# unilight/jatts

Hardware: AMD Instinct MI355X
Metric: audio samples/sec (22.05 kHz) + RTF, FastSpeech2+HiFi-GAN (higher is better)
Workload: dtype f32 (emulated: 3 exact bf16 terms per operand, 7 MFMA products, f32 accumulate; attention / norms / duration predictor exact f32); 1 GPU; FastSpeech2(JSUT conformer 4+4, adim 384)+HiFi-GAN v1 22k, 64 utts x 128 phonemes x 6 frames per GPU; hop=256, parallelism=dp1 (utterance sharding, int16 PCM all-gather)

## Files before the change

### jatts_amd/csrc/resunit_emul16_impl.h

```cpp
#pragma once
#include <type_traits>

#include "resunit_emul_impl.h"

#ifndef JATTS_U16_ROWS
#define JATTS_U16_ROWS 1
#endif
#ifndef JATTS_U16_DIAG
#define JATTS_U16_DIAG 0
#endif

namespace {

struct acc2x4 { f32x4 big, small; };
template <typename T> struct Acc16 { typedef f32x4 type; };
template <> struct Acc16<bf3p<7>> { typedef acc2x4 type; };
__device__ __forceinline__ void acc16_set(f32x4& a, int i, float v) { a[i] = v; }
__device__ __forceinline__ void acc16_set(acc2x4& a, int i, float v) { a.small[i] = v; a.big[i] = 0.f; }
__device__ __forceinline__ void acc16_finish(f32x4&) {}
__device__ __forceinline__ void acc16_finish(acc2x4& a) { a.small = a.big + a.small; }
__device__ __forceinline__ f32x4& acc16_val(f32x4& a) { return a; }
__device__ __forceinline__ f32x4& acc16_val(acc2x4& a) { return a.small; }

template <int P> __device__ __forceinline__ void mma16p(const bf3px8<7>& a, const bf3px8<7>& b, acc2x4& c) {
  if constexpr (P == 0) c.small = __builtin_amdgcn_mfma_f32_16x16x32_bf16(a.b1, b.b2, c.small, 0, 0, 0);
  if constexpr (P == 1) c.small = __builtin_amdgcn_mfma_f32_16x16x32_bf16(a.b2, b.b0, c.small, 0, 0, 0);
  if constexpr (P == 2) c.small = __builtin_amdgcn_mfma_f32_16x16x32_bf16(a.b0, b.b2, c.small, 0, 0, 0);
  if constexpr (P == 3) c.small = __builtin_amdgcn_mfma_f32_16x16x32_bf16(a.b1, b.b1, c.small, 0, 0, 0);
  if constexpr (P == 4) c.small = __builtin_amdgcn_mfma_f32_16x16x32_bf16(a.b1, b.b0, c.small, 0, 0, 0);
  if constexpr (P == 5) c.small = __builtin_amdgcn_mfma_f32_16x16x32_bf16(a.b0, b.b1, c.small, 0, 0, 0);
  if constexpr (P == 6) c.big = __builtin_amdgcn_mfma_f32_16x16x32_bf16(a.b0, b.b0, c.big, 0, 0, 0);
}
template <int P> __device__ __forceinline__ void mma16p(const bf3px8<6>& a, const bf3px8<6>& b, f32x4& c) {
  if constexpr (P == 0) c = __builtin_amdgcn_mfma_f32_16x16x32_bf16(a.b2, b.b0, c, 0, 0, 0);
  if constexpr (P == 1) c = __builtin_amdgcn_mfma_f32_16x16x32_bf16(a.b0, b.b2, c, 0, 0, 0);
  if constexpr (P == 2) c = __builtin_amdgcn_mfma_f32_16x16x32_bf16(a.b1, b.b1, c, 0, 0, 0);
  if constexpr (P == 3) c = __builtin_amdgcn_mfma_f32_16x16x32_bf16(a.b1, b.b0, c, 0, 0, 0);
  if constexpr (P == 4) c = __builtin_amdgcn_mfma_f32_16x16x32_bf16(a.b0, b.b1, c, 0, 0, 0);
  if constexpr (P == 5) c = __builtin_amdgcn_mfma_f32_16x16x32_bf16(a.b0, b.b0, c, 0, 0, 0);
}
template <typename T> struct NProd;
template <int NP> struct NProd<bf3p<NP>> { static constexpr int value = NP; };

template <typename T, int NF>
struct WStream16 {
  typedef typename Elem<T>::vec8 V8;
  V8 ra[NF];
  const T* wl;
  int kc_stride;
  int tap_stride;
  __device__ __forceinline__ void bind(const T* w, int KC32, int NFR16, int nf0, int lane) {
    wl = w + (size_t)nf0 * 512 + (size_t)lane * 8;
    kc_stride = NFR16 * 512;
    tap_stride = KC32 * kc_stride;
  }
  __device__ __forceinline__ void fetch(int tap, int kc) {
    const T* p = wl + (size_t)tap * tap_stride + (size_t)kc * kc_stride;
#pragma unroll
    for (int f = 0; f < NF; ++f) ra[f] = Vec8IO<T>::ldg(p + f * 512);
  }
};

template <typename T, int NF, int NT>
__device__ __forceinline__ void pair16(typename Acc16<T>::type (&acc)[NF][NT], const typename Elem<T>::vec8& a, typename Elem<T>::vec8 (&rb)[NT], int f_, int t0_) {
  constexpr int NP = NProd<T>::value;
  auto& c0 = acc[f_][t0_];
  auto& c1 = acc[f_][t0_ + 1];
  mma16p<0>(a, rb[t0_], c0); mma16p<0>(a, rb[t0_ + 1], c1);
  mma16p<1>(a, rb[t0_], c0); mma16p<1>(a, rb[t0_ + 1], c1);
  mma16p<2>(a, rb[t0_], c0); mma16p<2>(a, rb[t0_ + 1], c1);
  mma16p<3>(a, rb[t0_], c0); mma16p<3>(a, rb[t0_ + 1], c1);
  mma16p<4>(a, rb[t0_], c0); mma16p<4>(a, rb[t0_ + 1], c1);
  mma16p<5>(a, rb[t0_], c0); mma16p<5>(a, rb[t0_ + 1], c1);
  if constexpr (NP == 7) { mma16p<6>(a, rb[t0_], c0); mma16p<6>(a, rb[t0_ + 1], c1); }
}

template <typename T, int NF, int NT>
__device__ __forceinline__ void row16(typename Acc16<T>::type (&acc)[NF][NT], const typename Elem<T>::vec8& a, typename Elem<T>::vec8 (&rb)[NT], int f_) {
  constexpr int NP = NProd<T>::value;
#pragma unroll
  for (int t = 0; t < NT; ++t) mma16p<0>(a, rb[t], acc[f_][t]);
#pragma unroll
  for (int t = 0; t < NT; ++t) mma16p<1>(a, rb[t], acc[f_][t]);
#pragma unroll
  for (int t = 0; t < NT; ++t) mma16p<2>(a, rb[t], acc[f_][t]);
#pragma unroll
  for (int t = 0; t < NT; ++t) mma16p<3>(a, rb[t], acc[f_][t]);
#pragma unroll
  for (int t = 0; t < NT; ++t) mma16p<4>(a, rb[t], acc[f_][t]);
#pragma unroll
  for (int t = 0; t < NT; ++t) mma16p<5>(a, rb[t], acc[f_][t]);
  if constexpr (NP == 7) {
#pragma unroll
    for (int t = 0; t < NT; ++t) mma16p<6>(a, rb[t], acc[f_][t]);
  }
}

template <typename T, int NF, int NT>
__device__ __forceinline__ void step16(typename Acc16<T>::type (&acc)[NF][NT], typename Elem<T>::vec8 (&ra)[NF], typename Elem<T>::vec8 (&rb)[NT], const T* pa,
                                       const char* pb, int pitch) {
  static_assert(NT % 2 == 0, "column fragments come in pairs");
  constexpr bool ROWS16 = JATTS_U16_ROWS != 0;
#pragma unroll
  for (int f = 0; f < NF; ++f) {
    if (f < NF - 1 && ROWS16) {
      row16<T, NF, NT>(acc, ra[f], rb, f);
      __builtin_amdgcn_sched_barrier(0);
    } else {
#pragma unroll
      for (int tp = 0; tp < NT; tp += 2) {
        pair16<T, NF, NT>(acc, ra[f], rb, f, tp);
        if (f == NF - 1 && !(JATTS_U16_DIAG & 1)) {
          rb[tp] = Vec8IO<T>::lds(pb + (size_t)(tp * 16) * pitch);
          rb[tp + 1] = Vec8IO<T>::lds(pb + (size_t)((tp + 1) * 16) * pitch);
        }
        __builtin_amdgcn_sched_barrier(0);
      }
    }
    if (!(JATTS_U16_DIAG & 2)) ra[f] = Vec8IO<T>::ldg(pa + f * 512);
    __builtin_amdgcn_sched_barrier(0);
  }
}

template <typename T, int NF, int NT, int KCS>
__device__ __forceinline__ void conv16(typename Acc16<T>::type (&acc)[NF][NT], WStream16<T, NF>& ws, int kc0, int k_w, int dil, const char* act, int pitch,
                                       int col0, int lane, const T* tail) {
  typedef typename Elem<T>::vec8 V8;
  const int steps = k_w * KCS;
  const char* bbase = act + (size_t)(col0 + (lane & 15)) * pitch + (size_t)(lane >> 4) * 48;
  const T* abase = ws.wl + (size_t)kc0 * ws.kc_stride;
  V8 rb[NT];
#pragma unroll
  for (int t = 0; t < NT; ++t) rb[t] = Vec8IO<T>::lds(bbase + (size_t)(t * 16) * pitch);
  __builtin_amdgcn_sched_barrier(0);
  if (!tail) tail = abase + (size_t)(k_w - 1) * ws.tap_stride + (size_t)(KCS - 1) * ws.kc_stride;
  int tap = 0, kk = 0;
  for (int s = 0; s < steps; ++s) {
    int nkk = kk + 1;
    const bool wrap = nkk == KCS;
    nkk = wrap ? 0 : nkk;
    const int ntap = tap + (wrap ? 1 : 0);
    const bool last = s + 1 >= steps;
    const T* pa = last ? tail : abase + (size_t)ntap * ws.tap_stride + (size_t)nkk * ws.kc_stride;
    const char* pb = bbase + (size_t)((last ? tap : ntap) * dil) * pitch + (size_t)((last ? kk : nkk) * 4) * 48;
    step16<T, NF, NT>(acc, ws.ra, rb, pa, pb, pitch);
    tap = ntap;
    kk = nkk;
  }
}

template <typename T, int C, int WGCOLS, int WN, int WT, int OCC, bool KSPLIT = false, bool RREG = false, bool SLIDE = false>
__global__ __launch_bounds__(WN* WT * 64, OCC) void resunit_emul16_kernel(jatts_resunit_desc d, unsigned long long* trace, unsigned trace_cap,
                                                                         unsigned bias_off) {
  typedef typename Elem<T>::vec8 V8;
  extern __shared__ __attribute__((aligned(16))) char smem[];
  constexpr int NF = C / (WN * 16), NT = WGCOLS / (WT * 16);
  constexpr int KC32 = C / 32, NFR16 = C / 16;
  constexpr int pitch = C * 6 + 16;
  constexpr int pitch_x = KSPLIT ? (C / 2) * 6 + 16 : pitch;
  constexpr int pitch_t = C * 6;
  constexpr int NTHR = WN * WT * 64;
  static_assert(NF * WN * 16 == C && NT * WT * 16 == WGCOLS && C % 32 == 0, "tile shape");
  static_assert(sizeof(T) == 6, "bf3 is three packed bf16");
  static_assert(!(KSPLIT && RREG), "the residual registers go with the one-piece x tile");
  static_assert(!KSPLIT || KC32 % 2 == 0, "channel halves are whole K-steps");
  constexpr int MAXI = RREG ? (WGCOLS * (C / 8) + NTHR - 1) / NTHR : 1;
  f32x8 xk[MAXI];
  JATTS_TRACE_BEGIN(trace, trace_cap, blockIdx.x + blockIdx.y * gridDim.x);
  const int K = d.k_w, dil = d.dil;
  const int p2 = (K - 1) / 2, p1 = p2 * dil;
  const int tt_out = WGCOLS - 2 * p2;

  int b, t0;
  int64_t f_seq = 0, f_end = 0;
  if constexpr (!SLIDE) {
    int bx = blockIdx.x;
    b = blockIdx.y;
    if (ragged_is_1d(d.rg) && !ragged_locate(d.rg, tt_out, blockIdx.x, b, bx)) return;
    t0 = bx * tt_out;
  } else {
    const int c0 = d.rg.cu_rows[0];
    const int64_t total = (int64_t)(d.rg.cu_rows[d.rg.n_seq] - c0) * d.rg.len_mul;
    const int64_t per = (total + gridDim.x - 1) / gridDim.x;
    const int64_t f = (int64_t)blockIdx.x * per;
    if (f >= total) return;
    f_end = min(total, f + per);
    b = find_seq(d.rg.cu_rows, d.rg.n_seq, c0 + (int)(f / d.rg.len_mul));
    f_seq = (int64_t)(d.rg.cu_rows[b] - c0) * d.rg.len_mul;
    t0 = (int)(f - f_seq);
  }
  const int lane = threadIdx.x & 63, wave = threadIdx.x >> 6;
  const int wn = wave / WT, wt = wave % WT;
  const int g4 = lane >> 4;
  const int col0 = wt * NT * 16;
  const int nf0 = wn * NF;

  const int rx = WGCOLS + 2 * p1;
  char* xs = smem;
  char* hs = smem;
  float* bs = reinterpret_cast<float*>(smem + bias_off);
  char* tl = smem + bias_off - (SLIDE ? (K - 1) * pitch_t : 0);
  for (int u = threadIdx.x; u < 2 * C; u += NTHR) bs[u] = u < C ? d.b1[u] : d.b2[u - C];

  WStream16<T, NF> ws;
  typename Acc16<T>::type acc[NF][NT];
  auto bias_acc = [&](const float* bv) {
#pragma unroll
    for (int f = 0; f < NF; ++f) {
      const f32x4 bb = *reinterpret_cast<const f32x4*>(bv + (nf0 + f) * 16 + 4 * g4);
#pragma unroll
      for (int t = 0; t < NT; ++t)
#pragma unroll
        for (int e = 0; e < 4; ++e) acc16_set(acc[f][t], e, bb[e]);
    }
  };
  auto finish_acc = [&]() {
#pragma unroll
    for (int f = 0; f < NF; ++f)
#pragma unroll
      for (int t = 0; t < NT; ++t) acc16_finish(acc[f][t]);
  };
  auto to_planes = [&](f32x8 v) {
    lrelu8(v, d.slope);
    V8 o;
    bf3_split8(v, o);
    return o;
  };
  const float* x = (const float*)d.x;
  bool slide = false;
  for (bool first = true;; first = false) {
    unsigned tid = threadIdx.x;
    if constexpr (SLIDE) asm volatile("" : "+v"(tid));
    const int row_b = d.rg.cu_rows[b];
    const int L = (d.rg.cu_rows[b + 1] - row_b) * d.rg.len_mul;
    if constexpr (!SLIDE) {
      if (t0 >= L) return;
    }
    const int64_t seq_row0 = (int64_t)row_b * d.rg.len_mul;
    const int off = slide ? 2 * p2 : 0;
    const int nout = slide ? WGCOLS : tt_out;
    int nvalid = min(nout, L - t0);
    if constexpr (SLIDE) {
      nvalid = (int)min((int64_t)nvalid, f_end - f_seq - t0);
      if (!first) __syncthreads();
    }

    ws.bind((const T*)d.w1, KC32, NFR16, nf0, lane);
    ws.fetch(0, 0);
    const int pos0 = t0 - p2 + off - p1;
    if constexpr (!KSPLIT) {
      constexpr int UPR = C / 8;
      constexpr int UB = 8;
      const int total = rx * UPR;
      if constexpr (RREG) {
        const int r_in = p1 + p2 - off, n_in = nout * UPR;
#pragma unroll
        for (int j = 0; j < MAXI; ++j) {
          const int v = tid + j * NTHR;
          const int ro = v / UPR, cu = v - ro * UPR;
          const int pos = t0 + ro;
          if (v < n_in && pos < L) xk[j] = Vec8IO<float>::ldg(x + (seq_row0 + pos) * (int64_t)C + cu * 8);
          else xk[j] = f32x8{0, 0, 0, 0, 0, 0, 0, 0};
        }
        const int n_halo = (rx - nout) * UPR;
        for (int base = tid; base < n_halo; base += NTHR * UB) {
          f32x8 v[UB];
#pragma unroll
          for (int j = 0; j < UB; ++j) {
            const int u = base + j * NTHR;
            int r = u / UPR;
            const int cu = u - r * UPR;
            if (r >= r_in) r += nout;
            const int pos = pos0 + r;
            if (u < n_halo && pos >= 0 && pos < L) v[j] = Vec8IO<float>::ldg(x + (seq_row0 + pos) * (int64_t)C + cu * 8);
            else v[j] = f32x8{0, 0, 0, 0, 0, 0, 0, 0};
          }
#pragma unroll
          for (int j = 0; j < UB; ++j) {
            const int u = base + j * NTHR;
            if (u >= n_halo) continue;
            int r = u / UPR;
            const int cu = u - r * UPR;
            if (r >= r_in) r += nout;
            Vec8IO<T>::sts(xs + (size_t)r * pitch + (size_t)cu * 48, to_planes(v[j]));
          }
        }
#pragma unroll
        for (int j = 0; j < MAXI; ++j) {
          const int v = tid + j * NTHR;
          if (v >= n_in) continue;
          const int ro = v / UPR, cu = v - ro * UPR;
          Vec8IO<T>::sts(xs + (size_t)(r_in + ro) * pitch + (size_t)cu * 48, to_planes(xk[j]));
        }
      } else {
        constexpr int UBX = ((WGCOLS + 64) * UPR + NTHR - 1) / NTHR;
        for (int base = tid; base < total; base += NTHR * UBX) {
          f32x8 v[UBX];
#pragma unroll
          for (int j = 0; j < UBX; ++j) {
            const int u = base + j * NTHR;
            const int r = u / UPR, cu = u - r * UPR;
            const int pos = pos0 + r;
            if (u < total && pos >= 0 && pos < L) v[j] = Vec8IO<float>::ldg(x + (seq_row0 + pos) * (int64_t)C + cu * 8);
            else v[j] = f32x8{0, 0, 0, 0, 0, 0, 0, 0};
          }
#pragma unroll
          for (int j = 0; j < UBX; ++j) {
            const int u = base + j * NTHR;
            if (u >= total) continue;
            const int r = u / UPR, cu = u - r * UPR;
            Vec8IO<T>::sts(xs + (size_t)r * pitch + (size_t)cu * 48, to_planes(v[j]));
          }
        }
      }
      __syncthreads();
      JATTS_STAMP(2);
      bias_acc(bs);
      conv16<T, NF, NT, KC32>(acc, ws, 0, K, dil, xs, pitch, col0, lane, (const T*)d.w2 + (size_t)nf0 * 512 + (size_t)lane * 8);
    } else {
      constexpr int UPR = C / 16;
      constexpr int MAXU = ((WGCOLS + 64) * UPR + NTHR - 1) / NTHR;
      const int total = rx * UPR;
      f32x8 xv[MAXU];
      auto load_half = [&](int half) {
#pragma unroll
        for (int j = 0; j < MAXU; ++j) {
          const int u = tid + j * NTHR;
          const int r = u / UPR, cu = u - r * UPR;
          const int pos = pos0 + r;
          if (u < total && pos >= 0 && pos < L) xv[j] = Vec8IO<float>::ldg(x + (seq_row0 + pos) * (int64_t)C + half * (C / 2) + cu * 8);
          else xv[j] = f32x8{0, 0, 0, 0, 0, 0, 0, 0};
        }
      };
      auto store_half = [&]() {
#pragma unroll
        for (int j = 0; j < MAXU; ++j) {
          const int u = tid + j * NTHR;
          if (u < total) Vec8IO<T>::sts(xs + (size_t)(u / UPR) * pitch_x + (size_t)(u % UPR) * 48, to_planes(xv[j]));
        }
      };
      load_half(0);
      store_half();
      load_half(1);
      __syncthreads();
      JATTS_STAMP(2);
      bias_acc(bs);
      conv16<T, NF, NT, KC32 / 2>(acc, ws, 0, K, dil, xs, pitch_x, col0, lane, ws.wl + (size_t)(KC32 / 2) * ws.kc_stride);
      lds_barrier();
      store_half();
      lds_barrier();
      conv16<T, NF, NT, KC32 / 2>(acc, ws, KC32 / 2, K, dil, xs, pitch_x, col0, lane, (const T*)d.w2 + (size_t)nf0 * 512 + (size_t)lane * 8);
    }
    finish_acc();
    JATTS_STAMP(3);

    lds_barrier();
    JATTS_STAMP(10);
    if (SLIDE && slide) {
      for (int u = tid; u < (K - 1) * (C / 8); u += NTHR) {
        const int r = u / (C / 8), cu = u % (C / 8);
        Vec8IO<T>::sts(hs + (size_t)r * pitch + (size_t)cu * 48, Vec8IO<T>::lds(tl + (size_t)r * pitch_t + (size_t)cu * 48));
      }
    } else {
      for (int u = tid; u < (K - 1) * (C / 8); u += NTHR) {
        const int r = WGCOLS + u / (C / 8), cu = u % (C / 8);
        V8 z;
#pragma unroll
        for (int e = 0; e < 8; ++e) z.b0[e] = z.b1[e] = z.b2[e] = (bf16)0.f;
        Vec8IO<T>::sts(hs + (size_t)r * pitch + (size_t)cu * 48, z);
      }
    }
#pragma unroll
    for (int t = 0; t < NT; ++t) {
      const int col = col0 + t * 16 + (lane & 15);
      const int pos = t0 - p2 + off + col;
      const float keep = (pos >= 0 && pos < L) ? 1.f : 0.f;
#pragma unroll
      for (int f = 0; f < NF; ++f) {
        const int n0 = (nf0 + f) * 16 + 4 * g4;
        float v[4];
#pragma unroll
        for (int e = 0; e < 4; ++e) {
          const float a = acc16_val(acc[f][t])[e] * keep;
          v[e] = fmaxf(a, a * d.slope);
        }
        bf16x4 q0, q1, q2;
        bf3_split4(v, q0, q1, q2);
        char* p = hs + (size_t)(col + off) * pitch + (size_t)(n0 >> 3) * 48 + (size_t)(n0 & 4) * 2;
        *reinterpret_cast<bf16x4*>(p) = q0;
        *reinterpret_cast<bf16x4*>(p + 16) = q1;
        *reinterpret_cast<bf16x4*>(p + 32) = q2;
      }
    }
    JATTS_STAMP(12);
    lds_barrier();
    JATTS_STAMP(4);

    bias_acc(bs + C);
    ws.bind((const T*)d.w2, KC32, NFR16, nf0, lane);
    conv16<T, NF, NT, KC32>(acc, ws, 0, K, 1, hs, pitch, col0, lane, nullptr);
    finish_acc();
    JATTS_STAMP(5);

    __syncthreads();
    if constexpr (SLIDE) {
      for (int u = tid; u < (K - 1) * (C / 8); u += NTHR) {
        const int r = u / (C / 8), cu = u % (C / 8);
        Vec8IO<T>::sts(tl + (size_t)r * pitch_t + (size_t)cu * 48, Vec8IO<T>::lds(hs + (size_t)(nout + r) * pitch + (size_t)cu * 48));
      }
    }
    char* ys = smem;
#pragma unroll
    for (int t = 0; t < NT; ++t) {
      const int col = col0 + t * 16 + (lane & 15);
      if (col >= nvalid) continue;
#pragma unroll
      for (int f = 0; f < NF; ++f) {
        const int n0 = (nf0 + f) * 16 + 4 * g4;
        *reinterpret_cast<f32x4*>(ys + (size_t)col * pitch + (size_t)n0 * 4) = acc16_val(acc[f][t]);
      }
    }
    __syncthreads();
    JATTS_STAMP(6);
    {
      const int vrows = nvalid;
      const int64_t g0 = (seq_row0 + t0) * (int64_t)C;
      constexpr bool keep_small = C <= 64;
      const float* xg = (const float*)d.x;
      float* yg = (float*)d.y;
      if constexpr (RREG) {
        constexpr int UPR = C / 8;
        const int n_out = vrows * UPR;
        const bool has_add1 = d.add0 != nullptr && d.add1 != nullptr;
        f32x8 a0[MAXI], a1[MAXI];
        if (d.add0) {
#pragma unroll
          for (int j = 0; j < MAXI; ++j) {
            const int v = tid + j * NTHR;
            if (v < n_out) {
              a0[j] = Vec8IO<float>::ldg((const float*)d.add0 + g0 + (int64_t)v * 8);
              if (has_add1) a1[j] = Vec8IO<float>::ldg((const float*)d.add1 + g0 + (int64_t)v * 8);
            }
          }
        }
#pragma unroll
        for (int j = 0; j < MAXI; ++j) {
          const int v = tid + j * NTHR;
          if (v >= n_out) continue;
          const int ro = v / UPR, cu = v - ro * UPR;
          f32x8 o = Vec8IO<float>::lds(ys + (size_t)ro * pitch + (size_t)cu * 32);
#pragma unroll
          for (int e = 0; e < 8; ++e) o[e] = o[e] + xk[j][e];
          if (d.add0) {
#pragma unroll
            for (int e = 0; e < 8; ++e) o[e] = (o[e] + a0[j][e] + (has_add1 ? a1[j][e] : 0.f)) * d.out_scale;
          }
          float* dst = yg + g0 + (int64_t)v * 8;
          *reinterpret_cast<f32x4*>(dst) = f32x4{o[0], o[1], o[2], o[3]};
          *reinterpret_cast<f32x4*>(dst + 4) = f32x4{o[4], o[5], o[6], o[7]};
        }
      } else {
        if (d.add0) unit_store_pass<float, C, keep_small ? 2 : 4, true, NTHR>(d.add0, d.add1, d.out_scale, ys, pitch, vrows, xg, yg, g0);
        else unit_store_pass<float, C, keep_small ? 4 : 8, false, NTHR>(d.add0, d.add1, d.out_scale, ys, pitch, vrows, xg, yg, g0);
      }
    }
    JATTS_STAMP(7);
    if constexpr (!SLIDE) break;
    t0 += nout;
    slide = true;
    if (t0 >= L) {
      f_seq += L;
      if (f_seq >= f_end) break;
      do { ++b; } while (d.rg.cu_rows[b + 1] == d.rg.cu_rows[b]);
      t0 = 0;
      slide = false;
    } else if (f_seq + t0 >= f_end) {
      break;
    }
  }
  JATTS_TRACE_END();
}

inline int resunit16_pick(const jatts_resunit_desc& d, int runs, int wgcols, bool slide_auto, bool slide_fits) {
  const int64_t positions = ragged_is_1d(d.rg) ? (int64_t)d.rg.total_rows * d.rg.len_mul : (int64_t)d.rg.n_seq * d.rg.max_len * d.rg.len_mul;
  const bool slide = d.variant == 2 || (d.variant == 0 && slide_auto && positions >= 2 * (int64_t)runs * wgcols);
  return slide && slide_fits ? 2 : 1;
}

template <typename T, int C, int WGCOLS, int WN, int WT, int OCC = 2, bool KSPLIT = false, bool RREG = false>
int launch_resunit_emul16(const jatts_resunit_desc& d, hipStream_t s, int* pick) {
  const int K = d.k_w, p2 = (K - 1) / 2, p1 = p2 * d.dil;
  const int tt_out = WGCOLS - 2 * p2;
  if (tt_out < 8) return jatts_set_error_msg(JATTS_ERR_UNSUPPORTED, "resunit: kernel too wide for tile");
  const size_t pitch = C * 6 + 16, pitch_x = KSPLIT ? (C / 2) * 6 + 16 : pitch;
  const size_t rows_x = WGCOLS + 2 * p1, rows_h = WGCOLS + K - 1;
  if (KSPLIT && 2 * p1 > 64) return jatts_set_error_msg(JATTS_ERR_UNSUPPORTED, "resunit (emulated, channel halves): halo beyond 32 rows a side");
  const size_t region = rows_x * pitch_x > rows_h * pitch ? rows_x * pitch_x : rows_h * pitch;
  const size_t tail = (size_t)(K - 1) * C * 6;
  const size_t lds = region + 2 * C * sizeof(float);
  if (lds > 160 * 1024) return jatts_set_error_msg(JATTS_ERR_UNSUPPORTED, "resunit: tile exceeds 160 KiB LDS");
  int dev = 0, cus = 0;
  hipError_t e = hipGetDevice(&dev);
  if (e == hipSuccess) e = hipDeviceGetAttribute(&cus, hipDeviceAttributeMultiprocessorCount, dev);
  if (e != hipSuccess) return jatts_set_error(e, __FILE__, __LINE__);
  const int runs = cus * OCC;
  const int form = resunit16_pick(d, runs, WGCOLS, !RREG, lds + tail <= 160 * 1024);
  if (pick) {
    *pick = form;
    return JATTS_OK;
  }
  if (form == 2) {
    constexpr auto kern = resunit_emul16_kernel<T, C, WGCOLS, WN, WT, OCC, KSPLIT, RREG, true>;
    if (const int rc = unit_lds_ready<kern>(JATTS_SITE("resunit: tile exceeds 160 KiB LDS"), lds + tail)) return rc;
    hipLaunchKernelGGL(kern, dim3((unsigned)runs), dim3(WN * WT * 64), lds + tail, s, d, jatts_g_trace, jatts_g_trace_cap, (unsigned)(region + tail));
    JATTS_CHECK_LAUNCH();
    return JATTS_OK;
  }
  constexpr auto kern = resunit_emul16_kernel<T, C, WGCOLS, WN, WT, OCC, KSPLIT, RREG>;
  return unit_launch<kern>(JATTS_SITE("resunit: tile exceeds 160 KiB LDS"), WN * WT * 64, lds, tt_out, d.rg, s, d, jatts_g_trace, jatts_g_trace_cap, (unsigned)region);
}

}
```

Baseline: 67.15 million samples/s.

## Use buffer loads/stores with OOB zeroing and register-resident residual in resunit16

Replaces global loads and stores in the emulated 16x16 resunit kernel with raw buffer loads and stores on per-sequence resources, so out-of-range rows read as zero without per-element bounds branches. It adds a fused leaky-ReLU plus bf16 three-plane split, a fast path for the interior (non-edge) hidden-tile write, and an early prefetch of the residual input into registers before the second conv. The epilogue is rewritten so each thread works on fixed row strides. The new paths are skipped for one parent configuration (6-product, C=64, 128 columns), and a 2 GiB per-sequence limit check is added because buffer offsets are 32-bit.

After: 67.76 million samples/s, median of 6. Within noise of the previous version (+0.9%).

```diff
diff --git a/jatts_amd/csrc/resunit_emul16_impl.h b/jatts_amd/csrc/resunit_emul16_impl.h
--- a/jatts_amd/csrc/resunit_emul16_impl.h
+++ b/jatts_amd/csrc/resunit_emul16_impl.h
@@ -148,6 +148,65 @@
     kk = nkk;
   }
 }
+
+
+__device__ __forceinline__ float lrelu16(float v, float slope) {
+  const float m = v * slope;
+  float r;
+  asm("v_max_f32 %0, %1, %2" : "=v"(r) : "v"(v), "v"(m));
+  return r;
+}
+template <bool ASM2>
+__device__ __forceinline__ void bf3_split2p(f32x2 a, bf16x2& p0, bf16x2& p1, bf16x2& p2) {
+  p0 = __builtin_convertvector(a, bf16x2);
+  unsigned u = __builtin_bit_cast(unsigned, p0);
+  const f32x2 w0 = {__uint_as_float(u << 16), __uint_as_float(u & 0xffff0000u)};
+  const f32x2 r1 = a - w0;
+  p1 = __builtin_convertvector(r1, bf16x2);
+  u = __builtin_bit_cast(unsigned, p1);
+  const f32x2 w1 = {__uint_as_float(u << 16), __uint_as_float(u & 0xffff0000u)};
+  f32x2 r2 = r1 - w1;
+  if constexpr (ASM2) asm("v_pk_add_f32 %0, %1, %2 neg_lo:[0,1] neg_hi:[0,1]" : "=v"(r2) : "v"(r1), "v"(w1));
+  p2 = __builtin_convertvector(r2, bf16x2);
+}
+template <int NP>
+__device__ __forceinline__ bf3px8<NP> planes16(const f32x8& v, float slope) {
+  bf3px8<NP> o;
+#pragma unroll
+  for (int e = 0; e < 8; e += 2) {
+    bf16x2 p0, p1, p2;
+    bf3_split2p<false>(f32x2{lrelu16(v[e], slope), lrelu16(v[e + 1], slope)}, p0, p1, p2);
+    o.b0[e] = p0[0]; o.b0[e + 1] = p0[1];
+    o.b1[e] = p1[0]; o.b1[e + 1] = p1[1];
+    o.b2[e] = p2[0]; o.b2[e + 1] = p2[1];
+  }
+  return o;
+}
+
+constexpr unsigned kOOB16 = 0x80000000u;
+typedef unsigned u32x4_16 __attribute__((ext_vector_type(4)));
+__device__ __forceinline__ __amdgpu_buffer_rsrc_t seq_rsrc16(const void* p, unsigned bytes) {
+  const unsigned long long a = (unsigned long long)p;
+  const unsigned lo = __builtin_amdgcn_readfirstlane((unsigned)a), hi = __builtin_amdgcn_readfirstlane((unsigned)(a >> 32));
+  return __builtin_amdgcn_make_buffer_rsrc((void*)(((unsigned long long)hi << 32) | lo), 0, __builtin_amdgcn_readfirstlane(bytes), 0x00020000);
+}
+__device__ __forceinline__ f32x8 bld8(const __amdgpu_buffer_rsrc_t& r, unsigned voff) {
+  const f32x4 lo = __builtin_bit_cast(f32x4, __builtin_amdgcn_raw_buffer_load_b128(r, voff, 0, 0));
+  const f32x4 hi = __builtin_bit_cast(f32x4, __builtin_amdgcn_raw_buffer_load_b128(r, voff + 16, 0, 0));
+  return f32x8{lo[0], lo[1], lo[2], lo[3], hi[0], hi[1], hi[2], hi[3]};
+}
+__device__ __forceinline__ void loads_issued16() { asm volatile("" ::: "memory"); }
+__device__ __forceinline__ void bst8(const __amdgpu_buffer_rsrc_t& r, unsigned voff, const f32x8& o) {
+  __builtin_amdgcn_raw_buffer_store_b128(__builtin_bit_cast(u32x4_16, f32x4{o[0], o[1], o[2], o[3]}), r, voff, 0, 0);
+  __builtin_amdgcn_raw_buffer_store_b128(__builtin_bit_cast(u32x4_16, f32x4{o[4], o[5], o[6], o[7]}), r, voff + 16, 0, 0);
+}
+
+template <typename T, int C, int WGCOLS, bool KSPLIT, bool RREG, bool SLIDE>
+struct Phases16 {
+  static constexpr bool PARENT = NProd<T>::value == 6 && C == 64 && WGCOLS == 128;
+  static constexpr bool BUF = !PARENT, EDGE = !PARENT, STORE = !PARENT;
+  static constexpr bool PRE = STORE && !RREG;
+};
 
 template <typename T, int C, int WGCOLS, int WN, int WT, int OCC, bool KSPLIT = false, bool RREG = false, bool SLIDE = false>
 __global__ __launch_bounds__(WN* WT * 64, OCC) void resunit_emul16_kernel(jatts_resunit_desc d, unsigned long long* trace, unsigned trace_cap,
@@ -226,6 +285,15 @@
     bf3_split8(v, o);
     return o;
   };
+  typedef Phases16<T, C, WGCOLS, KSPLIT, RREG, SLIDE> PH;
+  constexpr int NPR = NProd<T>::value;
+  constexpr int UPRC = C / 8;
+  constexpr int RSTEP = NTHR / UPRC;
+  static_assert(NTHR % UPRC == 0 && WGCOLS % RSTEP == 0, "a thread's units lie in one column of units");
+  constexpr int NU = WGCOLS / RSTEP;
+  static_assert(!RREG || NU == MAXI, "the residual registers are the store pass's units");
+  constexpr unsigned ROWB = C * 4;
+  f32x8 xr[PH::PRE ? NU : 1];
   const float* x = (const float*)d.x;
   bool slide = false;
   for (bool first = true;; first = false) {
@@ -248,7 +316,55 @@
     ws.bind((const T*)d.w1, KC32, NFR16, nf0, lane);
     ws.fetch(0, 0);
     const int pos0 = t0 - p2 + off - p1;
-    if constexpr (!KSPLIT) {
+    const unsigned tr = tid / UPRC, tcu = tid % UPRC;
+    const unsigned seq_bytes = (unsigned)L * ROWB;
+    __amdgpu_buffer_rsrc_t rsx;
+    if constexpr (PH::BUF || PH::STORE) rsx = seq_rsrc16(x + seq_row0 * (int64_t)C, seq_bytes);
+    if constexpr (!KSPLIT && PH::BUF) {
+      const unsigned vx0 = (unsigned)(pos0 + (int)tr) * ROWB + tcu * 32;
+      char* const lx0 = xs + (size_t)tr * pitch + (size_t)tcu * 48;
+      if constexpr (RREG) {
+        const int r_in = p1 + p2 - off;
+        const unsigned vi0 = (unsigned)(t0 + (int)tr) * ROWB + tcu * 32;
+#pragma unroll
+        for (int j = 0; j < NU; ++j) xk[j] = bld8(rsx, (int)tr + j * RSTEP < nout ? vi0 + (unsigned)(j * RSTEP) * ROWB : kOOB16);
+        loads_issued16();
+        const int nh = rx - nout;
+        constexpr int UBH = 128 / RSTEP;
+        for (int hb = 0; hb < nh; hb += 128) {
+          f32x8 v[UBH];
+          int hr[UBH];
+#pragma unroll
+          for (int j = 0; j < UBH; ++j) {
+            const int h = hb + j * RSTEP + (int)tr;
+            hr[j] = h >= r_in ? h + nout : h;
+            v[j] = bld8(rsx, h < nh ? vx0 + (unsigned)hr[j] * ROWB - tr * ROWB : kOOB16);
+          }
+          loads_issued16();
+#pragma unroll
+          for (int j = 0; j < UBH; ++j)
+            if (hb + j * RSTEP + (int)tr < nh) Vec8IO<T>::sts(xs + (size_t)hr[j] * pitch + (size_t)tcu * 48, planes16<NPR>(v[j], d.slope));
+        }
+#pragma unroll
+        for (int j = 0; j < NU; ++j)
+          if ((int)tr + j * RSTEP < nout) Vec8IO<T>::sts(lx0 + (size_t)(r_in + j * RSTEP) * pitch, planes16<NPR>(xk[j], d.slope));
+      } else {
+        constexpr int UBX = (WGCOLS + 64 + RSTEP - 1) / RSTEP;
+        for (int rb0 = 0; rb0 < rx; rb0 += UBX * RSTEP) {
+          f32x8 v[UBX];
+#pragma unroll
+          for (int j = 0; j < UBX; ++j) v[j] = bld8(rsx, rb0 + j * RSTEP + (int)tr < rx ? vx0 + (unsigned)(rb0 + j * RSTEP) * ROWB : kOOB16);
+          loads_issued16();
+#pragma unroll
+          for (int j = 0; j < UBX; ++j)
+            if (rb0 + j * RSTEP + (int)tr < rx) Vec8IO<T>::sts(lx0 + (size_t)(rb0 + j * RSTEP) * pitch, planes16<NPR>(v[j], d.slope));
+        }
+      }
+      __syncthreads();
+      JATTS_STAMP(2);
+      bias_acc(bs);
+      conv16<T, NF, NT, KC32>(acc, ws, 0, K, dil, xs, pitch, col0, lane, (const T*)d.w2 + (size_t)nf0 * 512 + (size_t)lane * 8);
+    } else if constexpr (!KSPLIT) {
       constexpr int UPR = C / 8;
       constexpr int UB = 8;
       const int total = rx * UPR;
@@ -322,21 +438,38 @@
       constexpr int MAXU = ((WGCOLS + 64) * UPR + NTHR - 1) / NTHR;
       const int total = rx * UPR;
       f32x8 xv[MAXU];
+      constexpr int RSH = NTHR / UPR;
+      static_assert(NTHR % UPR == 0, "a thread's units lie in one column of units");
+      const unsigned hr0 = tid / UPR, hcu = tid % UPR;
       auto load_half = [&](int half) {
-#pragma unroll
-        for (int j = 0; j < MAXU; ++j) {
-          const int u = tid + j * NTHR;
-          const int r = u / UPR, cu = u - r * UPR;
-          const int pos = pos0 + r;
-          if (u < total && pos >= 0 && pos < L) xv[j] = Vec8IO<float>::ldg(x + (seq_row0 + pos) * (int64_t)C + half * (C / 2) + cu * 8);
-          else xv[j] = f32x8{0, 0, 0, 0, 0, 0, 0, 0};
+        if constexpr (PH::BUF) {
+          const unsigned v0 = (unsigned)(pos0 + (int)hr0) * ROWB + (unsigned)half * (C * 2) + hcu * 32;
+#pragma unroll
+          for (int j = 0; j < MAXU; ++j) xv[j] = bld8(rsx, (int)hr0 + j * RSH < rx ? v0 + (unsigned)(j * RSH) * ROWB : kOOB16);
+          loads_issued16();
+        } else {
+#pragma unroll
+          for (int j = 0; j < MAXU; ++j) {
+            const int u = tid + j * NTHR;
+            const int r = u / UPR, cu = u - r * UPR;
+            const int pos = pos0 + r;
+            if (u < total && pos >= 0 && pos < L) xv[j] = Vec8IO<float>::ldg(x + (seq_row0 + pos) * (int64_t)C + half * (C / 2) + cu * 8);
+            else xv[j] = f32x8{0, 0, 0, 0, 0, 0, 0, 0};
+          }
         }
       };
       auto store_half = [&]() {
-#pragma unroll
-        for (int j = 0; j < MAXU; ++j) {
-          const int u = tid + j * NTHR;
-          if (u < total) Vec8IO<T>::sts(xs + (size_t)(u / UPR) * pitch_x + (size_t)(u % UPR) * 48, to_planes(xv[j]));
+        if constexpr (PH::BUF) {
+          char* const l0 = xs + (size_t)hr0 * pitch_x + (size_t)hcu * 48;
+#pragma unroll
+          for (int j = 0; j < MAXU; ++j)
+            if ((int)hr0 + j * RSH < rx) Vec8IO<T>::sts(l0 + (size_t)(j * RSH) * pitch_x, planes16<NPR>(xv[j], d.slope));
+        } else {
+#pragma unroll
+          for (int j = 0; j < MAXU; ++j) {
+            const int u = tid + j * NTHR;
+            if (u < total) Vec8IO<T>::sts(xs + (size_t)(u / UPR) * pitch_x + (size_t)(u % UPR) * 48, to_planes(xv[j]));
+          }
         }
       };
       load_half(0);
@@ -370,6 +503,32 @@
         Vec8IO<T>::sts(hs + (size_t)r * pitch + (size_t)cu * 48, z);
       }
     }
+    if constexpr (PH::PRE) {
+      const unsigned vo0 = (unsigned)(t0 + (int)tr) * ROWB + tcu * 32;
+#pragma unroll
+      for (int i = 0; i < NU; ++i) xr[i] = bld8(rsx, vo0 + (unsigned)(i * RSTEP) * ROWB);
+      loads_issued16();
+    }
+    const int hpos0 = t0 - p2 + off;
+    const bool h_edge = !PH::EDGE || __builtin_amdgcn_readfirstlane((int)(hpos0 < 0 || hpos0 + WGCOLS > L)) != 0;
+    if (PH::EDGE && !h_edge) {
+#pragma unroll
+      for (int t = 0; t < NT; ++t) {
+        const int col = col0 + t * 16 + (lane & 15);
+        char* const pc = hs + (size_t)(col + off) * pitch + (size_t)(g4 >> 1) * 48 + (size_t)(g4 & 1) * 8;
+#pragma unroll
+        for (int f = 0; f < NF; ++f) {
+          const f32x4& a = acc16_val(acc[f][t]);
+          bf16x2 q0[2], q1[2], q2[2];
+          bf3_split2p<true>(f32x2{lrelu16(a[0], d.slope), lrelu16(a[1], d.slope)}, q0[0], q1[0], q2[0]);
+          bf3_split2p<true>(f32x2{lrelu16(a[2], d.slope), lrelu16(a[3], d.slope)}, q0[1], q1[1], q2[1]);
+          char* p = pc + (size_t)(nf0 + f) * 96;
+          *reinterpret_cast<bf16x4*>(p) = bf16x4{q0[0][0], q0[0][1], q0[1][0], q0[1][1]};
+          *reinterpret_cast<bf16x4*>(p + 16) = bf16x4{q1[0][0], q1[0][1], q1[1][0], q1[1][1]};
+          *reinterpret_cast<bf16x4*>(p + 32) = bf16x4{q2[0][0], q2[0][1], q2[1][0], q2[1][1]};
+        }
+      }
+    } else {
 #pragma unroll
     for (int t = 0; t < NT; ++t) {
       const int col = col0 + t * 16 + (lane & 15);
@@ -392,6 +551,7 @@
         *reinterpret_cast<bf16x4*>(p + 32) = q2;
       }
     }
+    }
     JATTS_STAMP(12);
     lds_barrier();
     JATTS_STAMP(4);
@@ -422,7 +582,58 @@
     }
     __syncthreads();
     JATTS_STAMP(6);
-    {
+    if constexpr (PH::STORE) {
+      const unsigned out_bytes = (unsigned)(t0 + nvalid) * ROWB;
+      const int64_t s0 = seq_row0 * (int64_t)C;
+      const __amdgpu_buffer_rsrc_t rsy = seq_rsrc16((float*)d.y + s0, out_bytes);
+      const unsigned vo0 = (unsigned)(t0 + (int)tr) * ROWB + tcu * 32;
+      const char* const ly0 = ys + (size_t)tr * pitch + (size_t)tcu * 32;
+      const bool has_add0 = d.add0 != nullptr, has_add1 = has_add0 && d.add1 != nullptr;
+      if (!has_add0) {
+        constexpr int UB = RREG || PH::PRE ? NU : (C <= 64 ? 4 : 8);
+#pragma unroll
+        for (int i0 = 0; i0 < NU; i0 += UB) {
+          f32x8 xb[RREG || PH::PRE ? 1 : UB];
+          if constexpr (!RREG && !PH::PRE) {
+#pragma unroll
+            for (int i = 0; i < UB; ++i) xb[i] = bld8(rsx, vo0 + (unsigned)((i0 + i) * RSTEP) * ROWB);
+          }
+#pragma unroll
+          for (int i = 0; i < UB; ++i) {
+            f32x8 o = Vec8IO<float>::lds(ly0 + (size_t)((i0 + i) * RSTEP) * pitch);
+            const f32x8& xv = RREG ? xk[RREG ? i0 + i : 0] : PH::PRE ? xr[PH::PRE ? i0 + i : 0] : xb[RREG || PH::PRE ? 0 : i];
+#pragma unroll
+            for (int e = 0; e < 8; ++e) o[e] = o[e] + xv[e];
+            bst8(rsy, vo0 + (unsigned)((i0 + i) * RSTEP) * ROWB, o);
+          }
+        }
+      } else {
+        const __amdgpu_buffer_rsrc_t rs0 = seq_rsrc16((const float*)d.add0 + s0, out_bytes);
+        const __amdgpu_buffer_rsrc_t rs1 = seq_rsrc16((const float*)(has_add1 ? d.add1 : d.add0) + s0, has_add1 ? out_bytes : 0u);
+        constexpr int UB = RREG ? NU : (C <= 64 ? 2 : 4);
+#pragma unroll
+        for (int i0 = 0; i0 < NU; i0 += UB) {
+          f32x8 xb[RREG || PH::PRE ? 1 : UB], a0[UB], a1[UB];
+#pragma unroll
+          for (int i = 0; i < UB; ++i) {
+            const unsigned vo = vo0 + (unsigned)((i0 + i) * RSTEP) * ROWB;
+            if constexpr (!RREG && !PH::PRE) xb[i] = bld8(rsx, vo);
+            a0[i] = bld8(rs0, vo);
+            if (has_add1) a1[i] = bld8(rs1, vo);
+          }
+#pragma unroll
+          for (int i = 0; i < UB; ++i) {
+            f32x8 o = Vec8IO<float>::lds(ly0 + (size_t)((i0 + i) * RSTEP) * pitch);
+            const f32x8& xv = RREG ? xk[RREG ? i0 + i : 0] : PH::PRE ? xr[PH::PRE ? i0 + i : 0] : xb[RREG || PH::PRE ? 0 : i];
+#pragma unroll
+            for (int e = 0; e < 8; ++e) o[e] = o[e] + xv[e];
+#pragma unroll
+            for (int e = 0; e < 8; ++e) o[e] = (o[e] + a0[i][e] + (has_add1 ? a1[i][e] : 0.f)) * d.out_scale;
+            bst8(rsy, vo0 + (unsigned)((i0 + i) * RSTEP) * ROWB, o);
+          }
+        }
+      }
+    } else {
       const int vrows = nvalid;
       const int64_t g0 = (seq_row0 + t0) * (int64_t)C;
       constexpr bool keep_small = C <= 64;
@@ -499,6 +710,8 @@
   const size_t tail = (size_t)(K - 1) * C * 6;
   const size_t lds = region + 2 * C * sizeof(float);
   if (lds > 160 * 1024) return jatts_set_error_msg(JATTS_ERR_UNSUPPORTED, "resunit: tile exceeds 160 KiB LDS");
+  if ((int64_t)d.rg.max_len * d.rg.len_mul * C * 4 >= (int64_t)1 << 31)
+    return jatts_set_error_msg(JATTS_ERR_UNSUPPORTED, "resunit (emulated, 16x16x32): a sequence of 2 GiB or more (positions x channels x 4 bytes)");
   int dev = 0, cus = 0;
   hipError_t e = hipGetDevice(&dev);
   if (e == hipSuccess) e = hipDeviceGetAttribute(&cus, hipDeviceAttributeMultiprocessorCount, dev);
```
